# csiro-robotics/ohm

Measured on AMD Instinct MI355X. Metric: rays/sec integrated (occupancy), higher is better.
Workload: dtype f64

## Files before the change

ohm_amd/csrc/batch_run.h:

```cpp
#ifndef OHMHIP_BATCH_RUN_H
#define OHMHIP_BATCH_RUN_H

namespace
{
struct BatchRun
{
  ohmhip_map_t m;
  const double *d_rays;
  const float *d_intensities;
  const double *d_timestamps;
  uint32_t n_rays;
  unsigned ray_flags;
  hipStream_t s, f;
  const Event *tev;
  uint32_t ring;
  uint32_t next_info_index = 0;
  bool info_clean = false;
  uint32_t ray_blocks = 0, bin_rays_per_block = 0, bin_threads = 0, bin_blocks = 0, bin_tab_mask = 0;
  uint32_t batch_chunk_segments = 0;
  int mode = 0;
  bool stop_mode = false, occupancy_mode = false, ndt_mode = false, tsdf_mode = false;
  bool occ_inline = false;
  int ray_shift = 0;
  SecondaryLayers sec;
  int attempt = 0;
  uint32_t spec_seg_cap = 0, seg_cap = 0;
  bool speculated = false, bucket_hits = false;
  BatchInfo info;
  unsigned long long *keys_a = nullptr, *keys_b = nullptr, *events = nullptr;
  const unsigned long long *sorted = nullptr;
  uint32_t event_capacity = 0, n_events = 0;
  float *direct_occ = nullptr;
  uint32_t direct_segments = 0;
  uint32_t sort_covers = 0;
  bool batch_end_marked = false;
  bool events_speculated = false;
  uint32_t spec_events = 0;

  uint32_t walkLdsHits() const { return uint32_t(m->walk_half ? WalkHalf::kLdsHits : WalkFull::kLdsHits); }

  void mark(int k) { m->tev_mask[ring] = uint8_t(m->tev_mask[ring] | (1u << k)); }

  int prepare()
  {
    m->tev_mask[ring] = 0;
    m->tev_pre_walk[ring] = 0;
    m->info_index = (m->info_index + 1u) % 3u;
    next_info_index = (m->info_index + 1u) % 3u;
    info_clean = m->info_clean;
    m->info_clean = false;
    m->parity ^= 1u;
    ray_blocks = (n_rays + 255) / 256;
    bin_rays_per_block = m->bin_rays_per_block;
    bin_threads = kBinThreads;
    while (bin_rays_per_block > 128 && n_rays / bin_rays_per_block < 2 * m->walk_workgroups)
    {
      bin_rays_per_block /= 2;
    }
    bin_threads = std::min<uint32_t>(bin_threads, bin_rays_per_block);
    bin_blocks = (n_rays + bin_rays_per_block - 1) / bin_rays_per_block;
    bin_tab_mask = std::min<uint32_t>(kLtabSize, std::max<uint32_t>(256u, 2u * bin_rays_per_block)) - 1u;
    const uint64_t expected_segments = uint64_t(double(n_rays) * m->segments_per_ray);
    batch_chunk_segments = m->chunk_segments;
    const uint32_t chunk_floor = (n_rays <= 16384u) ? std::min<uint32_t>(m->min_chunk_segments, 512u) : m->min_chunk_segments;
    while (batch_chunk_segments > chunk_floor &&
           expected_segments / batch_chunk_segments < 3ull * m->walkSlots())
    {
      batch_chunk_segments /= 2;
    }
    mode = m->config.mode;
    stop_mode = mode == OHMHIP_MODE_OCCUPANCY && (ray_flags & OHMHIP_RF_STOP_ON_FIRST_OCCUPIED) != 0;
    occupancy_mode = mode == OHMHIP_MODE_OCCUPANCY && !stop_mode;
    ndt_mode = mode == OHMHIP_MODE_NDT_OM || mode == OHMHIP_MODE_NDT_TM;
    tsdf_mode = mode == OHMHIP_MODE_TSDF;
    if (ndt_mode)
    {
      ray_flags &= (OHMHIP_RF_END_POINT_AS_FREE | OHMHIP_RF_EXCLUDE_ORIGIN | OHMHIP_RF_EXCLUDE_RAY);
    }
    if (tsdf_mode)
    {
      ray_flags = OHMHIP_RF_END_POINT_AS_FREE;
    }
    ray_shift = occupancy_mode ? 0 : kEvRayShift;
    sec.traversal = tsdf_mode ? nullptr : static_cast<float *>(m->pool.layers[OHMHIP_LID_TRAVERSAL].get());
    sec.touch_time = tsdf_mode ? nullptr : static_cast<uint32_t *>(m->pool.layers[OHMHIP_LID_TOUCH_TIME].get());
    sec.incident = tsdf_mode ? nullptr : static_cast<uint32_t *>(m->pool.layers[OHMHIP_LID_INCIDENT].get());
    sec.timestamps = d_timestamps;
    sec.time_base = m->first_ray_time;
    occ_inline = occupancy_mode && !m->pool.layers[OHMHIP_LID_MEAN] && !sec.traversal && !sec.touch_time && !sec.incident &&
                 !m->pool.layers[OHMHIP_LID_INTENSITY] && !m->pool.layers[OHMHIP_LID_HIT_MISS];

    for (int p = 0; p < 2; ++p)
    {
      OHMHIP_CHECK(m->walks_buf[p].ensure(sizeof(RayWalk) * size_t(n_rays), false, s));
      OHMHIP_CHECK(m->wg_regions[p].ensure(sizeof(WgRegion) * size_t(bin_blocks) * kLtabSize, false, s));
      OHMHIP_CHECK(m->wg_region_count[p].ensure(sizeof(uint32_t) * size_t(bin_blocks), false, s));
    }
    if (occupancy_mode)
    {
      OHMHIP_CHECK(m->hit_keys_a.ensure(sizeof(unsigned long long) * size_t(n_rays), false, s));
      OHMHIP_CHECK(m->hit_keys_b.ensure(sizeof(unsigned long long) * size_t(n_rays), false, s));
      OHMHIP_CHECK(m->interval_counts.ensure(sizeof(uint32_t) * size_t(n_rays), true, s));
      size_t sort_bytes = 0;
      OHMHIP_CHECK(rocprim::radix_sort_keys<SortConfig>(nullptr, sort_bytes, static_cast<unsigned long long *>(m->hit_keys_a.ptr),
                                            static_cast<unsigned long long *>(m->hit_keys_b.ptr), size_t(n_rays),
                                            kHitRayBits, sortEndBit(m), s));
      OHMHIP_CHECK(m->sort_temp.ensure(sort_bytes, false, s));
    }
    return OHMHIP_OK;
  }

  void launchBin(bool bucket, uint32_t seg_capacity, unsigned long long *hit_keys)
  {
    if (bin_tab_mask < kLtabSmall)
    {
      hipExtLaunchKernelGGL(k_ray_bin<kLtabSmall>, dim3(bin_blocks), dim3(bin_threads), 0, s, nullptr, tev[1], 0, m->mc,
                            regionTable(m), batchScratch(m), static_cast<const RayWalk *>(batchWalks(m).ptr), n_rays,
                            static_cast<Segment *>(m->segments.ptr), seg_capacity, hit_keys, m->pool.d_hit_mask.get(), ray_shift,
                            bucket ? 1 : 0, bin_rays_per_block, bin_tab_mask);
    }
    else
    {
      hipExtLaunchKernelGGL(k_ray_bin<kLtabSize>, dim3(bin_blocks), dim3(bin_threads), 0, s, nullptr, tev[1], 0, m->mc,
                            regionTable(m), batchScratch(m), static_cast<const RayWalk *>(batchWalks(m).ptr), n_rays,
                            static_cast<Segment *>(m->segments.ptr), seg_capacity, hit_keys, m->pool.d_hit_mask.get(), ray_shift,
                            bucket ? 1 : 0, bin_rays_per_block, bin_tab_mask);
    }
    mark(1);
    m->tev_pre_walk[ring] = 1;
    m->bin_done_event = tev[1];
  }

  void launchRegionSort(uint32_t dense)
  {
    const unsigned long long *in = static_cast<const unsigned long long *>(m->hit_keys_a.ptr);
    unsigned long long *out = static_cast<unsigned long long *>(m->hit_keys_b.ptr);
    const bool need_dense = kSortSmallHits == 0 || dense > kSortSmallHits;
    if (need_dense)
    {
      hipExtLaunchKernelGGL((k_sort_region_hits<kSortRegionHits, kSortThreads>), dim3(2 * m->walk_workgroups),
                            dim3(kSortThreads), 0, s, nullptr, kSortSmallHits ? nullptr : tev[2].handle, 0, regionTable(m),
                            batchScratch(m), in, out, m->mc.region_voxels, kSortSmallHits);
    }
    if (kSortSmallHits)
    {
      hipExtLaunchKernelGGL((k_sort_region_hits<kSortSmallHits ? kSortSmallHits : 64u, kSortSmallThreads>),
                            dim3(8 * m->walk_workgroups), dim3(kSortSmallThreads), 0, s, nullptr, tev[2], 0,
                            regionTable(m), batchScratch(m), in, out, m->mc.region_voxels, 0u);
    }
    sort_covers = need_dense ? kSortRegionHits : kSortSmallHits;
    mark(2);
    m->tev_pre_walk[ring] = 2;
  }

  void launchDenseSort()
  {
    hipExtLaunchKernelGGL((k_sort_region_hits<kSortRegionHits, kSortThreads>), dim3(2 * m->walk_workgroups),
                          dim3(kSortThreads), 0, s, nullptr, tev[2], 0, regionTable(m), batchScratch(m),
                          static_cast<const unsigned long long *>(m->hit_keys_a.ptr),
                          static_cast<unsigned long long *>(m->hit_keys_b.ptr), m->mc.region_voxels, kSortSmallHits);
    sort_covers = kSortRegionHits;
  }

  int frontHalf()
  {
    if (m->batch_done_event[m->parity])
    {
      OHMHIP_CHECK(hipStreamWaitEvent(f, m->batch_done_event[m->parity], 0));
    }
    if (m->bin_done_event)
    {
      OHMHIP_CHECK(hipStreamWaitEvent(f, m->bin_done_event, 0));
    }
    if (attempt > 0 || !info_clean)
    {
      OHMHIP_CHECK(hipMemsetAsync(m->d_info + m->info_index, 0, sizeof(BatchInfo), f));
    }
    if (m->phase_timing)
    {
      OHMHIP_CHECK(hipEventRecord(tev[0], f));
      mark(0);
    }
    if (bin_tab_mask < kLtabSmall)
    {
      hipLaunchKernelGGL(k_ray_setup<kLtabSmall>, dim3(bin_blocks), dim3(bin_threads), 0, f, m->mc, regionTable(m),
                         batchScratch(m), d_rays, n_rays, ray_flags, static_cast<RayWalk *>(batchWalks(m).ptr),
                         bin_rays_per_block, bin_tab_mask);
    }
    else
    {
      hipLaunchKernelGGL(k_ray_setup<kLtabSize>, dim3(bin_blocks), dim3(bin_threads), 0, f, m->mc, regionTable(m),
                         batchScratch(m), d_rays, n_rays, ray_flags, static_cast<RayWalk *>(batchWalks(m).ptr),
                         bin_rays_per_block, bin_tab_mask);
    }
    hipExtLaunchKernelGGL(k_plan, dim3(1), dim3(1024), 0, f, nullptr, tev[5], 0, regionTable(m), batchScratch(m),
                          batchChunks(m), m->pool.chunk_capacity, batch_chunk_segments, m->h_info.dev,
                          m->d_info + next_info_index, batchEventCount(m), occ_inline ? walkLdsHits() : 0u);
    mark(5);
    m->info_clean = true;
    hipEvent_t plan_done = tev[5];
    if (m->spill_enabled)
    {
      OHMHIP_CHECK(queueUseStamps(m, f));
      OHMHIP_CHECK(hipEventRecord(m->ev[7], f));
      plan_done = m->ev[7];
    }
    OHMHIP_CHECK(hipStreamWaitEvent(s, plan_done, 0));
    if (m->phase_timing)
    {
      OHMHIP_CHECK(hipEventRecord(tev[6], s));
      mark(6);
    }
    spec_seg_cap = uint32_t(std::min<size_t>(m->segments.bytes / sizeof(Segment), 0xffffffffu));
    speculated = occupancy_mode && m->spec_bucket_ok && attempt == 0 && spec_seg_cap > 0;
    if (speculated)
    {
      launchBin(true, spec_seg_cap, static_cast<unsigned long long *>(m->hit_keys_a.ptr));
      launchRegionSort(m->spec_max_region_hits);
    }
    OHMHIP_CHECK(hipEventSynchronize(plan_done));
    OHMHIP_CHECK(hipGetLastError());
    info = *m->h_info;
    return OHMHIP_OK;
  }

  bool exhausted() const
  {
    return (info.error & (kErrSlotsFull | kErrHashFull)) || info.n_slots > m->pool.slot_capacity ||
           info.n_chunks > m->pool.chunk_capacity;
  }

  int resolveExhaustion(bool &retry)
  {
    retry = false;
    OHMHIP_CHECK(hipStreamSynchronize(s));
    m->spec_bucket_ok = false;
    const int err = growPool(m, info.n_slots, m->pool.slot_capacity * 2u, m->slots_committed);
    if (err)
    {
      const int rollback_err = rollbackTable(m);
      if (rollback_err)
      {
        return rollback_err;
      }
      if (err == OHMHIP_ERR_CAPACITY && m->spill_enabled && !(info.error & kErrHashFull) &&
          info.n_slots > m->slots_committed)
      {
        const uint64_t allowed = poolBudget(m).regions;
        const uint64_t wanted = uint64_t(info.n_slots);
        m->batch_exceeds_limit = wanted > allowed && wanted - allowed > m->slots_committed;
        if (wanted > allowed && wanted - allowed <= m->slots_committed)
        {
          const int evict_err = evictColdRegions(m, uint32_t(wanted - allowed));
          if (evict_err == OHMHIP_OK)
          {
            retry = true;
            return OHMHIP_OK;
          }
        }
      }
      return err;
    }
    retry = true;
    return OHMHIP_OK;
  }

  int commitRegions()
  {
    m->cache_misses += info.n_slots - m->slots_committed;
    m->cache_hits += info.n_touched - std::min(info.n_touched, info.n_slots - m->slots_committed);
    if (!m->spilled.empty())
    {
      OHMHIP_CHECK(readmitSpilledSlots(m, m->slots_committed, info.n_slots));
    }
    m->slots_committed = info.n_slots;
    if (speculated && (info.n_segments > spec_seg_cap || info.max_region_hits > kSortRegionHits))
    {
      OHMHIP_CHECK(hipStreamSynchronize(s));
      if (info.n_touched)
      {
// ... 520 lines not shown
```

ohm_amd/csrc/partition_impl.h:

```cpp
#ifndef OHMHIP_PARTITION_IMPL_H
#define OHMHIP_PARTITION_IMPL_H

namespace
{
constexpr int kRouteThreads = 256;
constexpr uint32_t kRouteMaxWorld = 64;

__global__ void __launch_bounds__(kRouteThreads)
  k_route_mask(MapConst mc, const double *__restrict__ rays, uint32_t n_rays, unsigned ray_flags,
               unsigned long long *__restrict__ masks, uint32_t *__restrict__ block_counts, uint32_t world,
               unsigned long long *__restrict__ visits_out)
{
  __shared__ uint32_t s_counts[kRouteMaxWorld];
  __shared__ unsigned long long s_visits;
  if (threadIdx.x < kRouteMaxWorld)
  {
    s_counts[threadIdx.x] = 0;
  }
  if (threadIdx.x == 0)
  {
    s_visits = 0;
  }
  __syncthreads();
  const uint32_t ray = blockIdx.x * kRouteThreads + threadIdx.x;
  unsigned long long mask = 0;
  unsigned long long visits = 0;
  if (ray < n_rays)
  {
    RayWalk rw;
    double start[3], end[3];
#pragma unroll
    for (int a = 0; a < 3; ++a)
    {
      start[a] = rays[size_t(ray) * 6 + a];
      end[a] = rays[size_t(ray) * 6 + 3 + a];
    }
    setupRay(mc, start, end, ray_flags, rw, ray);
    if (rw.flags & kRwValid)
    {
      MapConst all = mc;
      all.owner_world = 0;
      forEachSegment(all, rw, false, [&](uint64_t key, const SegmentEntry &) { mask |= 1ull << regionOwnerOf(mc, key); });
      if (rw.flags & kRwApplySample)
      {
        uint64_t key;
        uint32_t vi;
        sampleVoxel(mc, rw, key, vi);
        mask |= 1ull << regionOwnerOf(mc, key);
      }
      const int manhattan = rw.total[0] + rw.total[1] + rw.total[2];
      if (rw.flags & kRwWalk)
      {
        visits += (unsigned long long)manhattan;
        visits -= ((rw.flags & kRwExcludeStart) && manhattan > 0) ? 1u : 0u;
        visits += (rw.flags & kRwIncludeEnd) ? 1u : 0u;
      }
      visits += (rw.flags & kRwApplySample) ? 1u : 0u;
    }
    masks[ray] = mask;
  }
  for (uint32_t d = 0; d < world; ++d)
  {
    const unsigned long long b = __ballot((mask >> d) & 1ull);
    if ((threadIdx.x & 63u) == 0 && b)
    {
      atomicAdd(&s_counts[d], uint32_t(__popcll(b)));
    }
  }
  if (visits)
  {
    atomicAdd(&s_visits, visits);
  }
  __syncthreads();
  if (threadIdx.x < world)
  {
    block_counts[size_t(threadIdx.x) * gridDim.x + blockIdx.x] = s_counts[threadIdx.x];
  }
  if (threadIdx.x == 0 && s_visits)
  {
    atomicAdd(visits_out, s_visits);
  }
}

__global__ void __launch_bounds__(1024)
  k_route_scan(uint32_t *__restrict__ block_counts, uint32_t n_blocks, uint32_t *__restrict__ totals,
               uint32_t *__restrict__ host_totals)
{
  __shared__ uint32_t s_wave[16];
  __shared__ uint32_t s_base;
  uint32_t *counts = block_counts + size_t(blockIdx.x) * n_blocks;
  if (threadIdx.x == 0)
  {
    s_base = 0;
  }
  __syncthreads();
  for (uint32_t first = 0; first < n_blocks; first += 1024)
  {
    const uint32_t i = first + threadIdx.x;
    const uint32_t c = (i < n_blocks) ? counts[i] : 0u;
    uint32_t incl = c;
#pragma unroll
    for (int d = 1; d < 64; d <<= 1)
    {
      const uint32_t up = __shfl_up(incl, d);
      incl += (int(threadIdx.x & 63u) >= d) ? up : 0u;
    }
    if ((threadIdx.x & 63u) == 63u)
    {
      s_wave[threadIdx.x >> 6] = incl;
    }
    __syncthreads();
    uint32_t before = 0, all = 0;
#pragma unroll
    for (uint32_t w = 0; w < 16; ++w)
    {
      const uint32_t v = s_wave[w];
      before += (w < (threadIdx.x >> 6)) ? v : 0u;
      all += v;
    }
    if (i < n_blocks)
    {
      counts[i] = s_base + before + incl - c;
    }
    __syncthreads();
    if (threadIdx.x == 0)
    {
      s_base += all;
    }
    __syncthreads();
  }
  if (threadIdx.x == 0)
  {
    totals[blockIdx.x] = s_base;
    host_totals[blockIdx.x] = s_base;
    __threadfence_system();
  }
}

__global__ void __launch_bounds__(kRouteThreads)
  k_route_scatter(const double *__restrict__ rays, uint32_t n_rays, const unsigned long long *__restrict__ masks,
                  const uint32_t *__restrict__ block_offsets, const uint32_t *__restrict__ totals, uint32_t world,
                  double *__restrict__ out_rays, uint32_t *__restrict__ out_index, uint32_t capacity)
{
  __shared__ uint32_t s_wave[kRouteThreads / 64];
  const uint32_t ray = blockIdx.x * kRouteThreads + threadIdx.x;
  const unsigned long long mask = (ray < n_rays) ? masks[ray] : 0ull;
  double r[6] = { 0, 0, 0, 0, 0, 0 };
  if (mask)
  {
#pragma unroll
    for (int a = 0; a < 6; ++a)
    {
      r[a] = rays[size_t(ray) * 6 + a];
    }
  }
  const unsigned lane = threadIdx.x & 63u;
  const unsigned wave = threadIdx.x >> 6;
  uint32_t dest_base = 0;
  for (uint32_t d = 0; d < world; ++d)
  {
    const bool mine = ((mask >> d) & 1ull) != 0;
    const unsigned long long b = __ballot(mine);
    if (lane == 0)
    {
      s_wave[wave] = uint32_t(__popcll(b));
    }
    __syncthreads();
    uint32_t before = 0;
    for (unsigned w = 0; w < wave; ++w)
    {
      before += s_wave[w];
    }
    __syncthreads();
    if (mine)
    {
      const uint32_t pos = dest_base + block_offsets[size_t(d) * gridDim.x + blockIdx.x] + before +
                           uint32_t(__popcll(b & ((1ull << lane) - 1ull)));
      if (pos < capacity)
      {
#pragma unroll
        for (int a = 0; a < 6; ++a)
        {
          out_rays[size_t(pos) * 6 + a] = r[a];
        }
        if (out_index)
        {
          out_index[pos] = ray;
        }
      }
    }
    dest_base += totals[d];
  }
}

uint32_t hostRegionOwner(ohmhip_map_t m, const int16_t *key)
// ... 349 lines not shown
```

ohm_amd/csrc/ray_front_kernels.h:

```cpp
#ifndef OHMHIP_RAY_FRONT_KERNELS_H
#define OHMHIP_RAY_FRONT_KERNELS_H

#include "batch_scratch.h"
#include "region_table.h"
#include "walk_device.h"

namespace ohmhip
{
struct RegionCursor
{
  int region[3];
  int next_j[3];
  int dir[3];
};

__device__ inline void regionCursorInit(const MapConst &mc, const RayWalk &rw, RegionCursor &rc)
{
#pragma unroll
  for (int a = 0; a < 3; ++a)
  {
    int local;
    splitGlobal(rw.g0[a], mc.dim[a], rc.region[a], local);
    rc.dir[a] = rwDir(rw, a);
    rc.next_j[a] = (rc.dir[a] > 0) ? (mc.dim[a] - local) : (local + 1);
  }
}

__device__ inline bool regionCursorNext(const MapConst &mc, const RayWalk &rw, RegionCursor &rc, int &axis, int &j)
{
  int best = -1;
  double best_t = 0;
#pragma unroll
  for (int a = 0; a < 3; ++a)
  {
    if (rc.next_j[a] <= rw.total[a])
    {
      const double t = stepTime(rw.init[a], rw.delta[a], rc.next_j[a]);
      if (best < 0 || stepPrecedes(t, a, best_t, best))
      {
        best = a;
        best_t = t;
      }
    }
  }
  if (best < 0)
  {
    return false;
  }
  axis = best;
  j = sel3(best, rc.next_j[0], rc.next_j[1], rc.next_j[2]);
  if (best == 0)
  {
    rc.region[0] += rc.dir[0];
    rc.next_j[0] += mc.dim[0];
  }
  else if (best == 1)
  {
    rc.region[1] += rc.dir[1];
    rc.next_j[1] += mc.dim[1];
  }
  else
  {
    rc.region[2] += rc.dir[2];
    rc.next_j[2] += mc.dim[2];
  }
  return true;
}

__device__ inline bool stepReachesEnd(const RayWalk &rw, int axis, int j)
{
  if (j != sel3(axis, rw.total[0], rw.total[1], rw.total[2]))
  {
    return false;
  }
  const double ta =
    stepTime(sel3(axis, rw.init[0], rw.init[1], rw.init[2]), sel3(axis, rw.delta[0], rw.delta[1], rw.delta[2]), j);
  bool all_before = true;
#pragma unroll
  for (int b = 0; b < 3; ++b)
  {
    if (rw.total[b] > 0)
    {
      const double tb = stepTime(rw.init[b], rw.delta[b], rw.total[b]);
      all_before = all_before && (b == axis || stepPrecedes(tb, b, ta, axis));
    }
  }
  return all_before;
}

struct SegmentEntry
{
  uint32_t k0 = 0, k1 = 0, k2 = 0;
  uint32_t count = 0;
  double t_base = 0;
  bool first = false;
  bool end = false;
};

template <typename F>
__device__ inline void forEachSegment(const MapConst &mc, const RayWalk &rw, bool with_resume_state, F emit)
{
  auto f = [&](uint64_t key, const SegmentEntry &entry) {
    if (ownsRegion(mc, key))
    {
      emit(key, entry);
    }
  };
  if (!(rw.flags & kRwValid) || !(rw.flags & kRwWalk))
  {
    return;
  }
  const int manhattan = rw.total[0] + rw.total[1] + rw.total[2];
  const bool include_end = (rw.flags & kRwIncludeEnd) != 0;
  RegionCursor rc;
  regionCursorInit(mc, rw, rc);
  bool have = false;
  uint64_t p_key = 0;
  SegmentEntry p;
  int p_sum = 0;
  if (manhattan > 0 || include_end)
  {
    p_key = packRegionKey(rc.region[0], rc.region[1], rc.region[2]);
    p.first = true;
    have = true;
    if (!with_resume_state)
    {
      f(p_key, p);
    }
  }
  double r0 = 0, r1 = 0, r2 = 0;
  if (with_resume_state)
  {
    r0 = 1.0 / rw.delta[0];
    r1 = 1.0 / rw.delta[1];
    r2 = 1.0 / rw.delta[2];
  }
  int axis, j;
  while (regionCursorNext(mc, rw, rc, axis, j))
  {
    if (stepReachesEnd(rw, axis, j) && !include_end)
    {
      continue;
    }
    const uint64_t key = packRegionKey(rc.region[0], rc.region[1], rc.region[2]);
    if (!with_resume_state)
    {
      f(key, p);
      continue;
    }
    const double ta = stepTime(sel3(axis, rw.init[0], rw.init[1], rw.init[2]),
                               sel3(axis, rw.delta[0], rw.delta[1], rw.delta[2]), j);
    const uint32_t rs0 = uint32_t((axis == 0) ? j : stepsBefore(rw.init[0], rw.delta[0], r0, rw.total[0], 0, axis, ta));
    const uint32_t rs1 = uint32_t((axis == 1) ? j : stepsBefore(rw.init[1], rw.delta[1], r1, rw.total[1], 1, axis, ta));
    const uint32_t rs2 = uint32_t((axis == 2) ? j : stepsBefore(rw.init[2], rw.delta[2], r2, rw.total[2], 2, axis, ta));
    const int sum = int(rs0 + rs1 + rs2);
    if (have)
    {
      p.count = uint32_t(sum - p_sum);
      f(p_key, p);
    }
    p_key = key;
    p.k0 = rs0;
    p.k1 = rs1;
    p.k2 = rs2;
    p.t_base = ta;
    p.first = false;
    p_sum = sum;
    have = true;
  }
  if (have && with_resume_state)
  {
    p.count = uint32_t(manhattan - p_sum) + (include_end ? 1u : 0u);
    p.end = include_end;
    f(p_key, p);
  }
}

struct RayFix
{
  uint32_t e0, e1, e2;
  bool poison;
};

__device__ inline RayFix rayFix(const MapConst &mc, const RayWalk &rw)
{
  RayFix rf;
  rf.poison = false;
  double t_last = 0;
  double t_phantom = dInf();
  uint32_t e[3];
#pragma unroll
  for (int a = 0; a < 3; ++a)
  {
    e[a] = 0;
    if (rw.total[a] > 0)
    {
      const double ex = rw.delta[a] * mc.fix_scale;
      rf.poison = rf.poison || !(ex >= 1.0);
      e[a] = !(ex >= 1.0) ? 0u : ((ex >= double(kFixMaxDelta)) ? kFixMaxDelta : uint32_t(ex));
      const double tl = stepTime(rw.init[a], rw.delta[a], rw.total[a]);
      const double tp = rw.init[a] + rw.delta[a] * double(rw.total[a]);
      rf.poison = rf.poison || !(tl * mc.fix_scale > -1.0) || !(tp >= tl);
      t_last = (tl > t_last) ? tl : t_last;
      t_phantom = (tp < t_phantom) ? tp : t_phantom;
    }
    e[a] |= rwSign(rw, a) ? kSegNegative : 0u;
  }
  rf.poison = rf.poison || !(t_phantom >= t_last);
  rf.e0 = e[0];
  rf.e1 = e[1];
  rf.e2 = e[2];
  return rf;
}

__device__ inline bool fixTime(const MapConst &mc, double init, double delta, int total, uint32_t k, double t_base,
                               uint32_t &f)
{
  if (int(k) >= total)
  {
    f = kFixFar;
    return true;
  }
  const double t = (k == 0) ? init : init + delta * double(k);
  const double x = (t - t_base) * mc.fix_scale;
  const bool ok = x > -1.0;
  f = !(x >= 1.0) ? 0u : ((x >= double(kFixFar)) ? kFixFar : uint32_t(x));
  return ok;
}

__device__ inline Segment makeSegment(const MapConst &mc, const RayWalk &rw, const RayFix &rf, uint32_t ray,
                                      const SegmentEntry &en)
{
  Segment sg;
  bool ok = !rf.poison;
  ok = fixTime(mc, rw.init[0], rw.delta[0], rw.total[0], en.k0, en.t_base, sg.f[0]) && ok;
  ok = fixTime(mc, rw.init[1], rw.delta[1], rw.total[1], en.k1, en.t_base, sg.f[1]) && ok;
  ok = fixTime(mc, rw.init[2], rw.delta[2], rw.total[2], en.k2, en.t_base, sg.f[2]) && ok;
  sg.e[0] = (int(en.k0) < rw.total[0]) ? rf.e0 : (rf.e0 & kSegNegative);
  sg.e[1] = (int(en.k1) < rw.total[1]) ? rf.e1 : (rf.e1 & kSegNegative);
  sg.e[2] = (int(en.k2) < rw.total[2]) ? rf.e2 : (rf.e2 & kSegNegative);
  if (!ok)
  {
    sg.f[0] = sg.f[1] = sg.f[2] = 0;
    sg.e[0] &= kSegNegative;
    sg.e[1] &= kSegNegative;
    sg.e[2] &= kSegNegative;
  }
  const int l0 = localCoord(rw.g0[0] + rwDir(rw, 0) * int(en.k0), mc.dim[0]);
  const int l1 = localCoord(rw.g0[1] + rwDir(rw, 1) * int(en.k1), mc.dim[1]);
  const int l2 = localCoord(rw.g0[2] + rwDir(rw, 2) * int(en.k2), mc.dim[2]);
  const uint32_t vi = uint32_t(l0 + l1 * mc.dim[0] + l2 * mc.dim[0] * mc.dim[1]);
  sg.vox = vi | (en.count << kSegVoxelBits);
  sg.ray = ray | ((en.first && (rw.flags & kRwExcludeStart)) ? kSegSkipFirst : 0u) | (en.end ? kSegEnd : 0u);
  return sg;
}

__device__ inline void sampleVoxel(const MapConst &mc, const RayWalk &rw, uint64_t &region_key, uint32_t &vi)
{
  int r1[3], l1[3];
#pragma unroll
  for (int a = 0; a < 3; ++a)
  {
    splitGlobal(rw.g0[a] + rwDir(rw, a) * rw.total[a], mc.dim[a], r1[a], l1[a]);
  }
  region_key = packRegionKey(r1[0], r1[1], r1[2]);
  vi = uint32_t(l1[0] + l1[1] * mc.dim[0] + l1[2] * mc.dim[0] * mc.dim[1]);
}

constexpr uint32_t kRayOrderBins = 64;

struct RayOrder
{
  uint32_t bins[kRayOrderBins];
  uint16_t perm[kBinRaysPerBlock];
};

__device__ inline uint32_t rayExtentBin(const MapConst &mc, unsigned flags, const int total[3])
{
  if (!(flags & kRwValid) || !(flags & kRwWalk))
  {
    return 0;
  }
  const int max_dim = max(mc.dim[0], max(mc.dim[1], mc.dim[2]));
  const uint32_t manhattan = uint32_t(total[0] + total[1] + total[2]);
  return min(manhattan >> (31 - __clz(max_dim)), kRayOrderBins - 1u);
}

template <typename BinOf>
__device__ inline void buildRayOrder(RayOrder &order, uint32_t n_local, BinOf bin_of)
{
  if (threadIdx.x < kRayOrderBins)
  {
    order.bins[threadIdx.x] = 0;
  }
  __syncthreads();
  uint32_t my_bins[8];
#pragma unroll
  for (uint32_t k = 0; k < 8; ++k)
  {
    const uint32_t idx = threadIdx.x + k * blockDim.x;
    my_bins[k] = 0;
    if (idx < n_local)
    {
      my_bins[k] = kRayOrderBins - 1u - bin_of(k, idx);
      atomicAdd(&order.bins[my_bins[k]], 1u);
    }
  }
  __syncthreads();
  if (threadIdx.x < kRayOrderBins)
  {
    const uint32_t count = order.bins[threadIdx.x];
    uint32_t incl = count;
#pragma unroll
    for (int d = 1; d < int(kRayOrderBins); d <<= 1)
    {
      const uint32_t up = __shfl_up(incl, d);
      incl += (int(threadIdx.x) >= d) ? up : 0u;
    }
    order.bins[threadIdx.x] = incl - count;
  }
  __syncthreads();
#pragma unroll
  for (uint32_t k = 0; k < 8; ++k)
  {
    const uint32_t idx = threadIdx.x + k * blockDim.x;
    if (idx < n_local)
    {
      order.perm[atomicAdd(&order.bins[my_bins[k]], 1u)] = uint16_t(idx);
    }
  }
  __syncthreads();
}

template <uint32_t kTab>
__global__ void __launch_bounds__(kBinThreads) __attribute__((amdgpu_waves_per_eu(6, 8)))
  k_ray_setup(MapConst mc, RegionTable rt, BatchScratch bs, const double *__restrict__ rays, uint32_t n_rays,
              unsigned ray_flags, RayWalk *__restrict__ walks, uint32_t rays_per_block, uint32_t tab_mask)
{
  __shared__ LdsRegionTableT<kTab> tab;
  __shared__ unsigned long long s_visits;
  __shared__ uint32_t s_rays_ok;
  __shared__ uint32_t s_list_n;
  for (uint32_t i = threadIdx.x; i <= tab_mask; i += blockDim.x)
  {
    tab.keys[i] = 0;
    tab.count[i] = 0;
    tab.cursor[i] = 0;
  }
  if (threadIdx.x == 0)
  {
    s_visits = 0;
    s_rays_ok = 0;
    s_list_n = 0;
  }
  __syncthreads();

  const uint32_t first = blockIdx.x * rays_per_block;
  const uint32_t last = min(first + rays_per_block, n_rays);
  unsigned long long my_visits = 0;
  uint32_t my_ok = 0;
  for (uint32_t ray = first + threadIdx.x; ray < last; ray += blockDim.x)
  {
    RayWalk rw;
    double start[3], end[3];
#pragma unroll
    for (int a = 0; a < 3; ++a)
    {
      start[a] = rays[size_t(ray) * 6 + a];
      end[a] = rays[size_t(ray) * 6 + 3 + a];
    }
    setupRay(mc, start, end, ray_flags, rw, ray);
    if (mc.owner_world > 1u && (rw.flags & kRwApplySample))
    {
      uint64_t sample_key;
      uint32_t sample_vi;
      sampleVoxel(mc, rw, sample_key, sample_vi);
      rw.flags &= ownsRegion(mc, sample_key) ? ~0u : ~unsigned(kRwApplySample);
    }
    walks[ray] = rw;
    my_ok += (rw.flags & kRwPassed) ? 1u : 0u;
    if (rw.flags & kRwBeyondTiles)
    {
      atomicAdd(&bs.info->n_beyond_tiles, 1u);
    }
    if (!(rw.flags & kRwValid))
    {
      continue;
    }
    const int manhattan = rw.total[0] + rw.total[1] + rw.total[2];
    if (rw.flags & kRwWalk)
    {
      my_visits += (unsigned long long)manhattan;
      my_visits -= ((rw.flags & kRwExcludeStart) && manhattan > 0) ? 1u : 0u;
      my_visits += (rw.flags & kRwIncludeEnd) ? 1u : 0u;
    }
    my_visits += (rw.flags & kRwApplySample) ? 1u : 0u;

    forEachSegment(mc, rw, false, [&](uint64_t key, const SegmentEntry &) {
      const uint32_t e = ltabFindOrInsert(tab, key, tab_mask);
      if (e < kLtabSize)
      {
        atomicAdd(&tab.count[e], 1u);
      }
      else
      {
        const uint32_t h = regionInsert(rt, key, &bs.info->error);
        atomicAdd(&bs.seg_count[h], 1u);
        markTouched(bs, h);
      }
    });
    if (rw.flags & kRwApplySample)
    {
      uint64_t key;
      uint32_t vi;
      sampleVoxel(mc, rw, key, vi);
      const uint32_t e = ltabFindOrInsert(tab, key, tab_mask);
      if (e < kLtabSize)
      {
        atomicAdd(&tab.cursor[e], 1u);
      }
      else
      {
        const uint32_t h = regionInsert(rt, key, &bs.info->error);
        atomicAdd(&bs.hit_count[h], 1u);
        markTouched(bs, h);
      }
    }
  }
  atomicAdd(&s_visits, my_visits);
  atomicAdd(&s_rays_ok, my_ok);
  __syncthreads();
  if (threadIdx.x == 0)
  {
    atomicAdd(&bs.info->visits, s_visits);
    atomicAdd(&bs.info->rays_ok, (unsigned long long)s_rays_ok);
  }
  for (uint32_t e = threadIdx.x; e <= tab_mask; e += blockDim.x)
  {
    const unsigned long long key = tab.keys[e];
    if (key)
    {
      const uint32_t h = regionInsert(rt, key, &bs.info->error);
      const uint32_t c = tab.count[e];
      if (c)
      {
        atomicAdd(&bs.seg_count[h], c);
      }
      markTouched(bs, h);
      const uint32_t hits = tab.cursor[e];
      if (hits)
      {
        atomicAdd(&bs.hit_count[h], hits);
      }
      WgRegion wr;
      wr.key = key;
      wr.count = c;
      wr.entry = e;
      wr.hash = h;
      wr.hits = hits;
      bs.wg_regions[size_t(blockIdx.x) * kLtabSize + atomicAdd(&s_list_n, 1u)] = wr;
    }
  }
  __syncthreads();
  if (threadIdx.x == 0)
  {
    bs.wg_region_count[blockIdx.x] = s_list_n;
  }
}

__global__ void __launch_bounds__(1024)
  k_plan(RegionTable rt, BatchScratch bs, Chunk *__restrict__ chunks, uint32_t chunk_capacity,
         uint32_t chunk_segments, BatchInfo *__restrict__ host_info, BatchInfo *__restrict__ next_info,
         uint32_t *__restrict__ event_count, uint32_t inline_max_hits)
{
  constexpr uint32_t kSizeClasses = 32;
  constexpr int kRounds = 4;
  constexpr uint32_t kBigQueue = 256;
  __shared__ uint32_t s_seg[16];
  __shared__ uint32_t s_chk[16];
  __shared__ uint32_t s_hit[16];
  __shared__ uint32_t s_seg_base;
  __shared__ uint32_t s_chk_base;
  __shared__ uint32_t s_hit_base;
  __shared__ uint32_t s_hit_max;
  __shared__ uint32_t s_class[kSizeClasses + 1];
  __shared__ uint32_t s_hclass[33];
  __shared__ uint32_t s_big_n;
  __shared__ uint32_t s_big[kBigQueue][4];
  __shared__ uint32_t s_n_apply_counts, s_n_apply_hits;
  const uint32_t n = bs.info->n_touched;
  const uint32_t tid = threadIdx.x;
  if (tid == 0)
  {
    s_seg_base = 0;
    s_chk_base = 0;
    s_hit_base = 0;
    s_hit_max = 0;
    s_big_n = 0;
    s_n_apply_counts = 0;
    s_n_apply_hits = 0;
  }
  if (tid <= kSizeClasses)
  {
    s_class[tid] = 0;
    s_hclass[tid] = 0;
  }
  __syncthreads();
  auto hitClass = [](uint32_t hits) { return uint32_t(32 - __clz(int(hits - 1u))) & 31u; };
  auto sizeClass = [&](uint32_t size) { return min(size * kSizeClasses / chunk_segments, kSizeClasses); };
  auto emit = [&](uint32_t h, uint32_t slot, uint32_t seg_excl, uint32_t cnt, uint32_t nchk, uint32_t per, uint32_t c) {
    const uint32_t begin = c * per;
    const uint32_t end = min(cnt, (c + 1) * per);
    const uint32_t pos = atomicAdd(&s_class[sizeClass(end - begin)], 1u);
    if (pos < chunk_capacity)
    {
      Chunk ch;
      ch.slot = slot;
      ch.seg_begin = seg_excl + begin;
      ch.seg_end = seg_excl + end;
      ch.hash_index = h | ((nchk == 1) ? 0x80000000u : 0u);
      chunks[pos] = ch;
    }
  };

  uint32_t r_h[kRounds], r_cnt[kRounds], r_slot[kRounds], r_off[kRounds], r_hits[kRounds];
  for (uint32_t base = 0, round = 0; base < n; base += 1024, ++round)
  {
    const uint32_t i = base + tid;
    uint32_t h = 0, cnt = 0, nchk = 0, slot = 0, hits = 0;
    if (i < n)
    {
      h = bs.touched[i];
      cnt = bs.seg_count[h];
      hits = bs.hit_count[h];
      slot = rt.vals[h];
      nchk = (cnt + chunk_segments - 1) / chunk_segments;
      if (hits)
      {
        atomicMax(&s_hit_max, hits);
        atomicAdd(&s_hclass[hitClass(hits)], 1u);
      }
      if (nchk > 1)
      {
        bs.apply_counts_list[atomicAdd(&s_n_apply_counts, 1u)] = h;
      }
      if (hits && (nchk != 1 || hits > inline_max_hits))
      {
        bs.apply_hits_list[atomicAdd(&s_n_apply_hits, 1u)] = h;
      }
    }
    uint32_t inc_seg = cnt, inc_chk = nchk, inc_hit = hits;
// ... 42 lines not shown
        touchRegionUse(bs.last_use, slot, bs.stamp);
      }
      if (nchk)
      {
        const uint32_t per = (cnt + nchk - 1) / nchk;
        if (nchk > 1)
        {
          atomicAdd(&s_class[sizeClass(per)], nchk - 1);
        }
        atomicAdd(&s_class[sizeClass(cnt - (nchk - 1) * per)], 1u);
      }
    }
#pragma unroll
    for (int k = 0; k < kRounds; ++k)
    {
      if (uint32_t(k) == round)
      {
        r_h[k] = h;
        r_cnt[k] = cnt;
        r_slot[k] = slot;
        r_off[k] = seg_excl;
        r_hits[k] = hits;
      }
    }
    __syncthreads();
    if (tid == 1023)
    {
      s_seg_base += all_seg;
      s_chk_base += all_chk;
      s_hit_base += all_hit;
    }
    __syncthreads();
  }
  if (tid == 0)
  {
    uint32_t run = 0;
    for (int c = int(kSizeClasses); c >= 0; --c)
    {
      const uint32_t count = s_class[c];
      s_class[c] = run;
      run += count;
    }
  }
  if (tid == 64)
  {
    uint32_t run = 0;
    for (int c = 31; c >= 0; --c)
    {
      const uint32_t count = s_hclass[c];
      s_hclass[c] = run;
      run += count;
    }
    s_hclass[32] = run;
  }
  __syncthreads();
  for (uint32_t base = 0, round = 0; base < n; base += 1024, ++round)
  {
    const uint32_t i = base + tid;
    uint32_t h = 0, cnt = 0, slot = 0, seg_excl = 0, hits = 0;
#pragma unroll
    for (int k = 0; k < kRounds; ++k)
    {
      if (uint32_t(k) == round)
      {
        h = r_h[k];
        cnt = r_cnt[k];
        slot = r_slot[k];
        seg_excl = r_off[k];
        hits = r_hits[k];
      }
    }
    if (round >= uint32_t(kRounds) && i < n)
    {
      h = bs.touched[i];
      cnt = bs.seg_count[h];
      slot = rt.vals[h];
      seg_excl = bs.seg_offset[h];
      hits = bs.hit_count[h];
    }
    if (i < n && hits)
    {
      bs.hit_count[h] = 0;
      bs.sort_list[atomicAdd(&s_hclass[hitClass(hits)], 1u)] = h;
    }
    const uint32_t nchk = (i < n) ? (cnt + chunk_segments - 1) / chunk_segments : 0u;
    if (nchk)
    {
      const uint32_t per = (cnt + nchk - 1) / nchk;
      uint32_t q = kBigQueue;
      if (nchk > 4)
      {
        q = atomicAdd(&s_big_n, 1u);
      }
      if (q < kBigQueue)
      {
        s_big[q][0] = h;
        s_big[q][1] = slot;
        s_big[q][2] = seg_excl;
        s_big[q][3] = cnt;
      }
      else
      {
        for (uint32_t c = 0; c < nchk; ++c)
        {
          emit(h, slot, seg_excl, cnt, nchk, per, c);
        }
      }
    }
  }
  __syncthreads();
  const uint32_t n_big = min(s_big_n, kBigQueue);
  for (uint32_t q = tid >> 6; q < n_big; q += 16)
  {
    const uint32_t cnt = s_big[q][3];
    const uint32_t nchk = (cnt + chunk_segments - 1) / chunk_segments;
    const uint32_t per = (cnt + nchk - 1) / nchk;
    for (uint32_t c = tid & 63u; c < nchk; c += 64)
    {
      emit(s_big[q][0], s_big[q][1], s_big[q][2], cnt, nchk, per, c);
    }
  }
  if (!(bs.info->error & (kErrSlotsFull | kErrHashFull)) && *rt.n_slots <= rt.slot_capacity && s_chk_base <= chunk_capacity)
  {
    for (uint32_t i = tid; i < n; i += 1024)
    {
      const uint32_t slot = rt.vals[bs.touched[i]];
      if (slot < rt.slot_capacity)
      {
        bs.dirty[slot] |= 7u;
      }
    }
  }
  if (tid == 0)
  {
    BatchInfo out = *bs.info;
    out.n_segments = s_seg_base;
    out.n_chunks = s_chk_base;
    out.n_slots = *rt.n_slots;
    out.n_hits = s_hit_base;
    out.max_region_hits = s_hit_max;
    out.n_hit_regions = s_hclass[32];
    out.n_apply_counts = s_n_apply_counts;
    out.n_apply_hits = s_n_apply_hits;
    *bs.info = out;
    *host_info = out;
    *next_info = BatchInfo{};
    event_count[0] = 0;
    event_count[1] = 0;
    event_count[3] = 0;
    __threadfence_system();
  }
}

template <uint32_t kTab>
__global__ void __launch_bounds__(kBinThreads)
  k_ray_bin(MapConst mc, RegionTable rt, BatchScratch bs, const RayWalk *__restrict__ walks, uint32_t n_rays,
            Segment *__restrict__ segments, uint32_t segment_capacity, unsigned long long *__restrict__ hit_keys,
            uint32_t *__restrict__ hit_mask, int ray_shift, int bucket_hits, uint32_t rays_per_block,
            uint32_t tab_mask)
{
  __shared__ LdsRegionTableT<kTab> tab;
  __shared__ uint32_t s_slot[kTab];
  if (bs.info->error & (kErrHashFull | kErrSlotsFull))
  {
    return;
  }
  for (uint32_t i = threadIdx.x; i <= tab_mask; i += blockDim.x)
  {
    tab.keys[i] = 0;
    tab.count[i] = 0;
    tab.cursor[i] = 0;
    s_slot[i] = kSlotUnassigned;
  }
  __syncthreads();

  const uint32_t first = blockIdx.x * rays_per_block;
  const uint32_t last = min(first + rays_per_block, n_rays);
  const uint32_t mask_words = uint32_t(mc.region_voxels + 31) >> 5;

  const uint32_t n_wg_regions = bs.wg_region_count[blockIdx.x];
  for (uint32_t i = threadIdx.x; i < n_wg_regions; i += blockDim.x)
  {
    const WgRegion wr = bs.wg_regions[size_t(blockIdx.x) * kLtabSize + i];
    tab.keys[wr.entry] = wr.key;
    if (wr.count)
    {
      tab.cursor[wr.entry] = bs.seg_offset[wr.hash] + atomicAdd(&bs.seg_cursor[wr.hash], wr.count);
    }
    if (wr.hits)
    {
      const uint32_t slot = rt.vals[wr.hash];
      s_slot[wr.entry] = slot;
      if (bucket_hits && slot < rt.slot_capacity)
      {
        tab.count[wr.entry] = atomicAdd(&bs.hit_end[slot], wr.hits);
      }
    }
  }
  __syncthreads();
  auto emitSample = [&](uint32_t ray, const RayWalk &rw) {
    unsigned long long hk = kHitInvalid;
    uint32_t pos = ray;
    if ((rw.flags & kRwValid) && (rw.flags & kRwApplySample))
    {
      uint64_t key;
      uint32_t vi;
      sampleVoxel(mc, rw, key, vi);
      const uint32_t e = ltabFind(tab, key, tab_mask);
      uint32_t slot;
      if (e < kLtabSize)
      {
        slot = s_slot[e];
        if (bucket_hits)
        {
          pos = atomicAdd(&tab.count[e], 1u);
        }
      }
      else
      {
        const uint32_t h = regionFind(rt, key);
        slot = (h != 0xffffffffu) ? rt.vals[h] : kSlotUnassigned;
        if (bucket_hits && slot < rt.slot_capacity)
        {
          pos = atomicAdd(&bs.hit_end[slot], 1u);
        }
      }
      if (slot < rt.slot_capacity)
      {
        hk = packHitKey(slot, vi, ray, ray_shift);
        atomicOr(&hit_mask[size_t(slot) * mask_words + (vi >> 5)], 1u << (vi & 31));
      }
    }
    if (!bucket_hits || hk != kHitInvalid)
    {
      hit_keys[pos] = hk;
    }
  };
  __shared__ RayOrder order;
  const uint32_t n_local = last - first;
  buildRayOrder(order, n_local, [&](uint32_t, uint32_t idx) {
    const RayWalk *w = walks + first + idx;
    const int total[3] = { w->total[0], w->total[1], w->total[2] };
    return rayExtentBin(mc, w->flags, total);
  });
  for (uint32_t idx = threadIdx.x; idx < n_local; idx += blockDim.x)
  {
    const uint32_t ray = first + order.perm[idx];
    const RayWalk rw = walks[ray];
    emitSample(ray, rw);
    const RayFix rf = rayFix(mc, rw);
    forEachSegment(mc, rw, true, [&](uint64_t key, const SegmentEntry &entry) {
      const uint32_t e = ltabFind(tab, key, tab_mask);
      uint32_t pos;
      if (e < kLtabSize)
      {
        pos = atomicAdd(&tab.cursor[e], 1u);
      }
      else
      {
        const uint32_t h = regionFind(rt, key);
        if (h == 0xffffffffu)
        {
          return;
        }
        pos = bs.seg_offset[h] + atomicAdd(&bs.seg_cursor[h], 1u);
      }
      if (pos < segment_capacity)
      {
        segments[pos] = makeSegment(mc, rw, rf, ray, entry);
      }
    });
  }
}

__global__ void __launch_bounds__(1024)
  k_count_passed(MapConst mc, const double *__restrict__ rays, uint32_t n_rays, unsigned ray_flags,
                 uint32_t *__restrict__ host_count)
{
  __shared__ uint32_t s_ok;
  if (threadIdx.x == 0)
  {
    s_ok = 0;
  }
  __syncthreads();
  uint32_t my_ok = 0;
  for (uint32_t ray = threadIdx.x; ray < n_rays; ray += blockDim.x)
  {
    RayWalk rw;
    double start[3], end[3];
#pragma unroll
    for (int a = 0; a < 3; ++a)
    {
      start[a] = rays[size_t(ray) * 6 + a];
      end[a] = rays[size_t(ray) * 6 + 3 + a];
    }
    setupRay(mc, start, end, ray_flags, rw, ray);
    my_ok += (rw.flags & kRwPassed) ? 1u : 0u;
  }
  atomicAdd(&s_ok, my_ok);
  __syncthreads();
  if (threadIdx.x == 0)
  {
    *host_count = s_ok;
  }
}

__global__ void __launch_bounds__(256)
  k_rekey_samples(MapConst mc, RegionTable rt, const RayWalk *__restrict__ walks, uint32_t n_rays,
                  unsigned long long *__restrict__ hit_keys, int ray_shift)
{
  const uint32_t ray = blockIdx.x * blockDim.x + threadIdx.x;
  if (ray >= n_rays)
  {
    return;
  }
  const RayWalk rw = walks[ray];
  unsigned long long hk = kHitInvalid;
  if ((rw.flags & kRwValid) && (rw.flags & kRwApplySample))
  {
    uint64_t key;
    uint32_t vi;
    sampleVoxel(mc, rw, key, vi);
    const uint32_t h = regionFind(rt, key);
    const uint32_t slot = (h != 0xffffffffu) ? rt.vals[h] : kSlotUnassigned;
    if (slot < rt.slot_capacity)
    {
      hk = packHitKey(slot, vi, ray, ray_shift);
    }
  }
  hit_keys[ray] = hk;
}
}

#endif
```

Baseline: 1.157 billion.

## Specialize ray-bin segment emission with fast step counts and power-of-two local coords

Splits the region walk into a simple key-only iterator for counting/routing and a dedicated bin iterator that builds Segment records on the fly. The bin path reuses the entry time from the region cursor, computes steps-before with a quick floor-based estimate, and falls back to the exact routine only near boundaries. It adds a template variant that uses bitmask local coordinates and skips ownership checks when the map is single-owner with power-of-two region dims. This is meant to cut the double-precision work per segment in k_ray_bin, at the cost of extra kernel instantiations and a tolerance-based fast path that must match the exact results.

Result: faster. 1.178 billion, median of 6 (+1.8%).

```diff
diff --git a/ohm_amd/csrc/batch_run.h b/ohm_amd/csrc/batch_run.h
--- a/ohm_amd/csrc/batch_run.h
+++ b/ohm_amd/csrc/batch_run.h
@@ -112,20 +112,15 @@
 
   void launchBin(bool bucket, uint32_t seg_capacity, unsigned long long *hit_keys)
   {
-    if (bin_tab_mask < kLtabSmall)
-    {
-      hipExtLaunchKernelGGL(k_ray_bin<kLtabSmall>, dim3(bin_blocks), dim3(bin_threads), 0, s, nullptr, tev[1], 0, m->mc,
-                            regionTable(m), batchScratch(m), static_cast<const RayWalk *>(batchWalks(m).ptr), n_rays,
-                            static_cast<Segment *>(m->segments.ptr), seg_capacity, hit_keys, m->pool.d_hit_mask.get(), ray_shift,
-                            bucket ? 1 : 0, bin_rays_per_block, bin_tab_mask);
-    }
-    else
-    {
-      hipExtLaunchKernelGGL(k_ray_bin<kLtabSize>, dim3(bin_blocks), dim3(bin_threads), 0, s, nullptr, tev[1], 0, m->mc,
-                            regionTable(m), batchScratch(m), static_cast<const RayWalk *>(batchWalks(m).ptr), n_rays,
-                            static_cast<Segment *>(m->segments.ptr), seg_capacity, hit_keys, m->pool.d_hit_mask.get(), ray_shift,
-                            bucket ? 1 : 0, bin_rays_per_block, bin_tab_mask);
-    }
+    const auto pow2 = [](int v) { return (v & (v - 1)) == 0; };
+    const bool plain = m->mc.owner_world <= 1u && pow2(m->mc.dim[0]) && pow2(m->mc.dim[1]) && pow2(m->mc.dim[2]);
+    const bool small = bin_tab_mask < kLtabSmall;
+    const auto kernel = small ? (plain ? k_ray_bin<kLtabSmall, true> : k_ray_bin<kLtabSmall, false>) :
+                                (plain ? k_ray_bin<kLtabSize, true> : k_ray_bin<kLtabSize, false>);
+    hipExtLaunchKernelGGL(kernel, dim3(bin_blocks), dim3(bin_threads), 0, s, nullptr, tev[1], 0, m->mc, regionTable(m),
+                          batchScratch(m), static_cast<const RayWalk *>(batchWalks(m).ptr), n_rays,
+                          static_cast<Segment *>(m->segments.ptr), seg_capacity, hit_keys, m->pool.d_hit_mask.get(), ray_shift,
+                          bucket ? 1 : 0, bin_rays_per_block, bin_tab_mask);
     mark(1);
     m->tev_pre_walk[ring] = 1;
     m->bin_done_event = tev[1];
diff --git a/ohm_amd/csrc/partition_impl.h b/ohm_amd/csrc/partition_impl.h
--- a/ohm_amd/csrc/partition_impl.h
+++ b/ohm_amd/csrc/partition_impl.h
@@ -40,7 +40,7 @@
     {
       MapConst all = mc;
       all.owner_world = 0;
-      forEachSegment(all, rw, false, [&](uint64_t key, const SegmentEntry &) { mask |= 1ull << regionOwnerOf(mc, key); });
+      forEachSegment(all, rw, [&](uint64_t key) { mask |= 1ull << regionOwnerOf(mc, key); });
       if (rw.flags & kRwApplySample)
       {
         uint64_t key;
diff --git a/ohm_amd/csrc/ray_front_kernels.h b/ohm_amd/csrc/ray_front_kernels.h
--- a/ohm_amd/csrc/ray_front_kernels.h
+++ b/ohm_amd/csrc/ray_front_kernels.h
@@ -26,7 +26,8 @@
   }
 }
 
-__device__ inline bool regionCursorNext(const MapConst &mc, const RayWalk &rw, RegionCursor &rc, int &axis, int &j)
+__device__ inline bool regionCursorNext(const MapConst &mc, const RayWalk &rw, RegionCursor &rc, int &axis, int &j,
+                                        double &t_entry)
 {
   int best = -1;
   double best_t = 0;
@@ -48,6 +49,7 @@
     return false;
   }
   axis = best;
+  t_entry = best_t;
   j = sel3(best, rc.next_j[0], rc.next_j[1], rc.next_j[2]);
   if (best == 0)
   {
@@ -67,14 +69,12 @@
   return true;
 }
 
-__device__ inline bool stepReachesEnd(const RayWalk &rw, int axis, int j)
+__device__ inline bool stepReachesEnd(const RayWalk &rw, int axis, int j, double ta)
 {
   if (j != sel3(axis, rw.total[0], rw.total[1], rw.total[2]))
   {
     return false;
   }
-  const double ta =
-    stepTime(sel3(axis, rw.init[0], rw.init[1], rw.init[2]), sel3(axis, rw.delta[0], rw.delta[1], rw.delta[2]), j);
   bool all_before = true;
 #pragma unroll
   for (int b = 0; b < 3; ++b)
@@ -88,22 +88,23 @@
   return all_before;
 }
 
-struct SegmentEntry
-{
-  uint32_t k0 = 0, k1 = 0, k2 = 0;
-  uint32_t count = 0;
-  double t_base = 0;
-  bool first = false;
-  bool end = false;
-};
+__device__ inline bool stepReachesEnd(const RayWalk &rw, int axis, int j)
+{
+  if (j != sel3(axis, rw.total[0], rw.total[1], rw.total[2]))
+  {
+    return false;
+  }
+  return stepReachesEnd(rw, axis, j, stepTime(sel3(axis, rw.init[0], rw.init[1], rw.init[2]),
+                                              sel3(axis, rw.delta[0], rw.delta[1], rw.delta[2]), j));
+}
 
 template <typename F>
-__device__ inline void forEachSegment(const MapConst &mc, const RayWalk &rw, bool with_resume_state, F emit)
-{
-  auto f = [&](uint64_t key, const SegmentEntry &entry) {
+__device__ inline void forEachSegment(const MapConst &mc, const RayWalk &rw, F emit)
+{
+  auto f = [&](uint64_t key) {
     if (ownsRegion(mc, key))
     {
-      emit(key, entry);
+      emit(key);
     }
   };
   if (!(rw.flags & kRwValid) || !(rw.flags & kRwWalk))
@@ -114,65 +115,19 @@
   const bool include_end = (rw.flags & kRwIncludeEnd) != 0;
   RegionCursor rc;
   regionCursorInit(mc, rw, rc);
-  bool have = false;
-  uint64_t p_key = 0;
-  SegmentEntry p;
-  int p_sum = 0;
   if (manhattan > 0 || include_end)
   {
-    p_key = packRegionKey(rc.region[0], rc.region[1], rc.region[2]);
-    p.first = true;
-    have = true;
-    if (!with_resume_state)
-    {
-      f(p_key, p);
-    }
-  }
-  double r0 = 0, r1 = 0, r2 = 0;
-  if (with_resume_state)
-  {
-    r0 = 1.0 / rw.delta[0];
-    r1 = 1.0 / rw.delta[1];
-    r2 = 1.0 / rw.delta[2];
+    f(packRegionKey(rc.region[0], rc.region[1], rc.region[2]));
   }
   int axis, j;
-  while (regionCursorNext(mc, rw, rc, axis, j))
+  double ta;
+  while (regionCursorNext(mc, rw, rc, axis, j, ta))
   {
     if (stepReachesEnd(rw, axis, j) && !include_end)
     {
       continue;
     }
-    const uint64_t key = packRegionKey(rc.region[0], rc.region[1], rc.region[2]);
-    if (!with_resume_state)
-    {
-      f(key, p);
-      continue;
-    }
-    const double ta = stepTime(sel3(axis, rw.init[0], rw.init[1], rw.init[2]),
-                               sel3(axis, rw.delta[0], rw.delta[1], rw.delta[2]), j);
-    const uint32_t rs0 = uint32_t((axis == 0) ? j : stepsBefore(rw.init[0], rw.delta[0], r0, rw.total[0], 0, axis, ta));
-    const uint32_t rs1 = uint32_t((axis == 1) ? j : stepsBefore(rw.init[1], rw.delta[1], r1, rw.total[1], 1, axis, ta));
-    const uint32_t rs2 = uint32_t((axis == 2) ? j : stepsBefore(rw.init[2], rw.delta[2], r2, rw.total[2], 2, axis, ta));
-    const int sum = int(rs0 + rs1 + rs2);
-    if (have)
-    {
-      p.count = uint32_t(sum - p_sum);
-      f(p_key, p);
-    }
-    p_key = key;
-    p.k0 = rs0;
-    p.k1 = rs1;
-    p.k2 = rs2;
-    p.t_base = ta;
-    p.first = false;
-    p_sum = sum;
-    have = true;
-  }
-  if (have && with_resume_state)
-  {
-    p.count = uint32_t(manhattan - p_sum) + (include_end ? 1u : 0u);
-    p.end = include_end;
-    f(p_key, p);
+    f(packRegionKey(rc.region[0], rc.region[1], rc.region[2]));
   }
 }
 
@@ -213,46 +168,129 @@
   return rf;
 }
 
-__device__ inline bool fixTime(const MapConst &mc, double init, double delta, int total, uint32_t k, double t_base,
-                               uint32_t &f)
-{
-  if (int(k) >= total)
-  {
-    f = kFixFar;
-    return true;
-  }
+__device__ inline uint32_t fixTime(const MapConst &mc, double init, double delta, int total, uint32_t k, double t_base,
+                                   bool &live, bool &ok)
+{
+  live = int(k) < total;
   const double t = (k == 0) ? init : init + delta * double(k);
   const double x = (t - t_base) * mc.fix_scale;
-  const bool ok = x > -1.0;
-  f = !(x >= 1.0) ? 0u : ((x >= double(kFixFar)) ? kFixFar : uint32_t(x));
-  return ok;
-}
-
-__device__ inline Segment makeSegment(const MapConst &mc, const RayWalk &rw, const RayFix &rf, uint32_t ray,
-                                      const SegmentEntry &en)
-{
-  Segment sg;
+  ok = ok && (!live || x > -1.0);
+  const uint32_t f = !(x >= 1.0) ? 0u : ((x >= double(kFixFar)) ? kFixFar : uint32_t(x));
+  return live ? f : kFixFar;
+}
+
+template <bool kPlain>
+__device__ inline void segmentHead(const MapConst &mc, const RayWalk &rw, const RayFix &rf, const RegionCursor &rc,
+                                   uint32_t k0, uint32_t k1, uint32_t k2, double t_base, Segment &sg)
+{
   bool ok = !rf.poison;
-  ok = fixTime(mc, rw.init[0], rw.delta[0], rw.total[0], en.k0, en.t_base, sg.f[0]) && ok;
-  ok = fixTime(mc, rw.init[1], rw.delta[1], rw.total[1], en.k1, en.t_base, sg.f[1]) && ok;
-  ok = fixTime(mc, rw.init[2], rw.delta[2], rw.total[2], en.k2, en.t_base, sg.f[2]) && ok;
-  sg.e[0] = (int(en.k0) < rw.total[0]) ? rf.e0 : (rf.e0 & kSegNegative);
-  sg.e[1] = (int(en.k1) < rw.total[1]) ? rf.e1 : (rf.e1 & kSegNegative);
-  sg.e[2] = (int(en.k2) < rw.total[2]) ? rf.e2 : (rf.e2 & kSegNegative);
-  if (!ok)
-  {
-    sg.f[0] = sg.f[1] = sg.f[2] = 0;
-    sg.e[0] &= kSegNegative;
-    sg.e[1] &= kSegNegative;
-    sg.e[2] &= kSegNegative;
-  }
-  const int l0 = localCoord(rw.g0[0] + rwDir(rw, 0) * int(en.k0), mc.dim[0]);
-  const int l1 = localCoord(rw.g0[1] + rwDir(rw, 1) * int(en.k1), mc.dim[1]);
-  const int l2 = localCoord(rw.g0[2] + rwDir(rw, 2) * int(en.k2), mc.dim[2]);
-  const uint32_t vi = uint32_t(l0 + l1 * mc.dim[0] + l2 * mc.dim[0] * mc.dim[1]);
-  sg.vox = vi | (en.count << kSegVoxelBits);
-  sg.ray = ray | ((en.first && (rw.flags & kRwExcludeStart)) ? kSegSkipFirst : 0u) | (en.end ? kSegEnd : 0u);
-  return sg;
+  bool live0, live1, live2;
+  const uint32_t f0 = fixTime(mc, rw.init[0], rw.delta[0], rw.total[0], k0, t_base, live0, ok);
+  const uint32_t f1 = fixTime(mc, rw.init[1], rw.delta[1], rw.total[1], k1, t_base, live1, ok);
+  const uint32_t f2 = fixTime(mc, rw.init[2], rw.delta[2], rw.total[2], k2, t_base, live2, ok);
+  sg.f[0] = ok ? f0 : 0u;
+  sg.f[1] = ok ? f1 : 0u;
+  sg.f[2] = ok ? f2 : 0u;
+  sg.e[0] = (ok && live0) ? rf.e0 : (rf.e0 & kSegNegative);
+  sg.e[1] = (ok && live1) ? rf.e1 : (rf.e1 & kSegNegative);
+  sg.e[2] = (ok && live2) ? rf.e2 : (rf.e2 & kSegNegative);
+  auto local = [&](int g0, int dir, uint32_t k, int dim) {
+    const int g = g0 + ((int(k) ^ (dir >> 1)) - (dir >> 1));
+    return kPlain ? (g & (dim - 1)) : localCoord(g, dim);
+  };
+  const int l0 = local(rw.g0[0], rc.dir[0], k0, mc.dim[0]);
+  const int l1 = local(rw.g0[1], rc.dir[1], k1, mc.dim[1]);
+  const int l2 = local(rw.g0[2], rc.dir[2], k2, mc.dim[2]);
+  sg.vox = uint32_t(l0 + l1 * mc.dim[0] + l2 * mc.dim[0] * mc.dim[1]);
+}
+
+__device__ inline bool stepsBeforeQuick(double init, double rdelta, int total, bool fast, double ta, int &n)
+{
+  const double x = (ta - init) * rdelta;
+  const double whole = floor(x);
+  const double frac = x - whole;
+  n = min(max(int(whole) + 1, 0), total);
+  return fast && frac > 1e-5 && frac < 1.0 - 1e-5 && fabs(x) < 1048576.0;
+}
+
+template <bool kPlain, typename F>
+__device__ inline void forEachBinSegment(const MapConst &mc, const RayWalk &rw, const RayFix &rf, uint32_t ray, F emit)
+{
+  if (!(rw.flags & kRwValid) || !(rw.flags & kRwWalk))
+  {
+    return;
+  }
+  const int manhattan = rw.total[0] + rw.total[1] + rw.total[2];
+  const bool include_end = (rw.flags & kRwIncludeEnd) != 0;
+  if (manhattan == 0 && !include_end)
+  {
+    return;
+  }
+  const bool all_mine = kPlain || mc.owner_world <= 1u;
+  auto f = [&](uint64_t key, const Segment &sg) {
+    if (all_mine || ownsRegion(mc, key))
+    {
+      emit(key, sg);
+    }
+  };
+  RegionCursor rc;
+  regionCursorInit(mc, rw, rc);
+  const double r0 = 1.0 / rw.delta[0];
+  const double r1 = 1.0 / rw.delta[1];
+  const double r2 = 1.0 / rw.delta[2];
+  bool fast[3];
+#pragma unroll
+  for (int a = 0; a < 3; ++a)
+  {
+    fast[a] = rw.total[a] != 0 && rw.delta[a] > 0 && rw.delta[a] < dInf() && fabs(rw.init[a]) <= 4.0 * rw.delta[a];
+  }
+  uint64_t p_key = packRegionKey(rc.region[0], rc.region[1], rc.region[2]);
+  Segment p;
+  segmentHead<kPlain>(mc, rw, rf, rc, 0u, 0u, 0u, 0.0, p);
+  p.ray = ray | ((rw.flags & kRwExcludeStart) ? kSegSkipFirst : 0u);
+  int p_sum = 0;
+  int axis, j;
+  double ta;
+    while (regionCursorNext(mc, rw, rc, axis, j, ta))
+  {
+    if (stepReachesEnd(rw, axis, j, ta) && !include_end)
+    {
+      continue;
+    }
+    const uint64_t key = packRegionKey(rc.region[0], rc.region[1], rc.region[2]);
+    int n0, n1, n2;
+    const bool exact0 = !stepsBeforeQuick(rw.init[0], r0, rw.total[0], fast[0], ta, n0) && rw.total[0] != 0 && axis != 0;
+    const bool exact1 = !stepsBeforeQuick(rw.init[1], r1, rw.total[1], fast[1], ta, n1) && rw.total[1] != 0 && axis != 1;
+    const bool exact2 = !stepsBeforeQuick(rw.init[2], r2, rw.total[2], fast[2], ta, n2) && rw.total[2] != 0 && axis != 2;
+    if (exact0 || exact1 || exact2)
+    {
+#pragma unroll 1
+      for (int b = 0; b < 3; ++b)
+      {
+        if (sel3(b, exact0, exact1, exact2))
+        {
+          const int n = stepsBefore(sel3(b, rw.init[0], rw.init[1], rw.init[2]), sel3(b, rw.delta[0], rw.delta[1], rw.delta[2]),
+                                    sel3(b, r0, r1, r2), sel3(b, rw.total[0], rw.total[1], rw.total[2]), b, axis, ta);
+          n0 = (b == 0) ? n : n0;
+          n1 = (b == 1) ? n : n1;
+          n2 = (b == 2) ? n : n2;
+        }
+      }
+    }
+    n0 = (axis == 0) ? j : n0;
+    n1 = (axis == 1) ? j : n1;
+    n2 = (axis == 2) ? j : n2;
+    const int sum = n0 + n1 + n2;
+    p.vox |= uint32_t(sum - p_sum) << kSegVoxelBits;
+    f(p_key, p);
+    p_key = key;
+    segmentHead<kPlain>(mc, rw, rf, rc, uint32_t(n0), uint32_t(n1), uint32_t(n2), ta, p);
+    p.ray = ray;
+    p_sum = sum;
+  }
+  p.vox |= (uint32_t(manhattan - p_sum) + (include_end ? 1u : 0u)) << kSegVoxelBits;
+  p.ray |= include_end ? kSegEnd : 0u;
+  f(p_key, p);
 }
 
 __device__ inline void sampleVoxel(const MapConst &mc, const RayWalk &rw, uint64_t &region_key, uint32_t &vi)
@@ -396,7 +434,7 @@
     }
     my_visits += (rw.flags & kRwApplySample) ? 1u : 0u;
 
-    forEachSegment(mc, rw, false, [&](uint64_t key, const SegmentEntry &) {
+    forEachSegment(mc, rw, [&](uint64_t key) {
       const uint32_t e = ltabFindOrInsert(tab, key, tab_mask);
       if (e < kLtabSize)
       {
@@ -745,7 +783,7 @@
   }
 }
 
-template <uint32_t kTab>
+template <uint32_t kTab, bool kPlain>
 __global__ void __launch_bounds__(kBinThreads)
   k_ray_bin(MapConst mc, RegionTable rt, BatchScratch bs, const RayWalk *__restrict__ walks, uint32_t n_rays,
             Segment *__restrict__ segments, uint32_t segment_capacity, unsigned long long *__restrict__ hit_keys,
@@ -842,7 +880,7 @@
     const RayWalk rw = walks[ray];
     emitSample(ray, rw);
     const RayFix rf = rayFix(mc, rw);
-    forEachSegment(mc, rw, true, [&](uint64_t key, const SegmentEntry &entry) {
+    forEachBinSegment<kPlain>(mc, rw, rf, ray, [&](uint64_t key, const Segment &sg) {
       const uint32_t e = ltabFind(tab, key, tab_mask);
       uint32_t pos;
       if (e < kLtabSize)
@@ -860,7 +898,7 @@
       }
       if (pos < segment_capacity)
       {
-        segments[pos] = makeSegment(mc, rw, rf, ray, entry);
+        segments[pos] = sg;
       }
     });
   }
```
